# Masthetheus/kmer-ml

Hardware: NVIDIA B200
Metric: kmer_count_feature_throughput (higher is better)
Workload: dtype u32

## Files before the change

### kmerml_b200/csrc/dense.cu

```cuda
#include <algorithm>

#include "fasta_walk.cuh"
#include "internal.h"

namespace km {

struct DevTails {
    const LevelMap* lm;
    GenomeStats* st;
    uint32_t genome;
    __device__ __noinline__ void tail(int j, uint32_t idx) const {
        atomicAdd(lm->ptr(genome, j) + idx, 1u);
        atomicAdd(&st->n_tail[j], 1ull);
    }
};

struct NoTails {
    __device__ __forceinline__ void tail(int, uint32_t) const {}
};

struct TailList {
    unsigned long long* list;
    unsigned int* counts;
    unsigned int* any_full;
// ... 477 lines not shown
    tails.lm = &lm; tails.st = stats + sl.genome; tails.genome = sl.genome;
    Packed16Sink sink;
    sink.sbase = (uint32_t)__cvta_generic_to_shared(sh_hist); sink.n = 0;
    uint32_t* row8 = lm.ptr(sl.genome, 8);
    walk_slice<true, COUNT8_THREADS>(buf, g, sl, P, sink, tails, tc,
                                     [&](uint32_t) { sweep_packed16<COUNT8_THREADS>(sh_hist, row8); });
    const unsigned long long total = block_sum_u32(sink.n, &sh_total);
    for (int i = tid; i < 32768; i += COUNT8_THREADS) packed16_flush_word(sh_hist[i], (uint32_t)i, row8);
    if (tid == 0 && total) atomicAdd(&stats[sl.genome].total_top, total);
}

constexpr int PART_LOW = 7;
constexpr int PART_BINS = 1 << (2 * PART_LOW);
constexpr int PART_MAX_BUCKETS = 1024;
constexpr int PART_SECTOR = 16;

__device__ __noinline__ void overflow_push(uint32_t* ov, unsigned int* ov_count, uint32_t idx) {
    const unsigned act = __activemask();
    const int lane = threadIdx.x & 31;
    const int leader = __ffs(act) - 1;
    unsigned int base = 0;
    if (lane == leader) base = atomicAdd(ov_count, (unsigned int)__popc(act));
    base = __shfl_sync(act, base, leader);
    ov[base + __popc(act & ((1u << lane) - 1u))] = idx;
}

__device__ __forceinline__ uint32_t payload_fix(uint32_t bucket) { return ((bucket & 3u) << 14) * 0x00010001u; }
__device__ __forceinline__ uint32_t payload_pad(uint32_t bucket, uint32_t spread) {
    return (((bucket & 3u) ^ 1u) << 14) | (spread & 255u);
}

__device__ __noinline__ void overflow_push_sector(uint32_t* ov, unsigned int* ov_count, uint32_t bucket,
                                                  const uint16_t* src) {
    for (int i = 0; i < PART_SECTOR; i++)
        overflow_push(ov, ov_count, (bucket << (2 * PART_LOW)) | (src[i] & (uint32_t)(PART_BINS - 1)));
}

template <int NB_SHIFT>
struct PartGeom {
    static constexpr uint32_t nb = 1u << NB_SHIFT;
    static constexpr uint32_t slot_size = NB_SHIFT == 10 ? 48u : (32768u >> NB_SHIFT);
    static constexpr uint32_t stage_entries = nb * slot_size;
    static constexpr bool owned = NB_SHIFT == 10;
};

template <int NB_SHIFT>
struct SlotSink {
    static constexpr bool raw_windows = true;
    static constexpr uint32_t slot_size = PartGeom<NB_SHIFT>::slot_size;
    static constexpr uint32_t b4_mask = (PartGeom<NB_SHIFT>::nb - 1u) << 2;
    uint32_t cnt_s;
    uint32_t staged_s;
    uint32_t* ov;
    unsigned int* ov_count;
    uint32_t kmask;
    unsigned n;
    __device__ __forceinline__ uint32_t atom_inc(uint32_t b4) {
        uint32_t old;
        asm volatile("atom.shared.add.u32 %0, [%1], 1;" : "=r"(old) : "r"(cnt_s + b4) : "memory");
        return old;
    }
    __device__ __forceinline__ void store16(uint32_t b4, uint32_t pos, uint32_t x) {
        const uint32_t e = b4 * (slot_size / 4u) + pos;
        asm volatile("st.shared.u16 [%0], %1;" ::"r"(staged_s + 2u * e), "h"((unsigned short)x) : "memory");
    }
    __device__ __forceinline__ void count(uint32_t idx, uint64_t) {
        const uint32_t b4 = (idx >> (2 * PART_LOW - 2)) & b4_mask;
        const uint32_t pos = atom_inc(b4);
        n++;
        if (pos < slot_size) store16(b4, pos, idx);
        else overflow_push(ov, ov_count, idx);
    }
    __device__ __forceinline__ void count4(uint32_t i0, uint32_t i1, uint32_t i2, uint32_t i3, uint64_t, uint64_t,
                                           uint64_t, uint64_t) {
        count(i0, 0); count(i1, 0); count(i2, 0); count(i3, 0);
    }
    __device__ __forceinline__ void count8(const uint32_t* w, const uint64_t*) { place<8>(w, true); }
    __device__ __forceinline__ void count8_tail(const uint32_t* w, const uint64_t*, bool last) { place<8>(w, last); }
    template <int N>
    __device__ __forceinline__ void place(const uint32_t* x, bool last_live = true) {
        uint32_t b4[N], pos[N];
        bool full = false;
#pragma unroll
        for (int u = 0; u < N; u++) b4[u] = (x[u] >> (2 * PART_LOW - 2)) & b4_mask;
#pragma unroll
        for (int u = 0; u < N; u++) pos[u] = (u < N - 1 || last_live) ? atom_inc(b4[u]) : 0u;
        n += last_live ? N : N - 1;
#pragma unroll
        for (int u = 0; u < N; u++) {
            const bool fits = pos[u] < slot_size;
            full |= !fits;
            if (fits && (u < N - 1 || last_live)) store16(b4[u], pos[u], x[u]);
        }
        if (full) {
#pragma unroll
            for (int u = 0; u < N; u++)
                if (pos[u] >= slot_size) overflow_push(ov, ov_count, x[u] & kmask);
        }
    }
};

struct PartWalkSmem {
    uint32_t last16[COUNT_THREADS];
    uint8_t flags[2 * COUNT_THREADS];
    uint8_t clean[COUNT_THREADS];
};

template <int NB_SHIFT>
struct PartSmem {
    uint16_t staged[PartGeom<NB_SHIFT>::stage_entries];
    uint32_t cnt[PART_MAX_BUCKETS];
    uint16_t written[PART_MAX_BUCKETS];
    PartWalkSmem walk;
    unsigned long long carry[2];
    uint32_t prev_tile[2];
    unsigned long long sh_total;
};
static_assert(sizeof(PartSmem<10>) <= 113 * 1024, "two partition CTAs must fit in one SM's shared memory");

struct GenomeRuns {
    uint32_t run0, n_runs;
};

__device__ __forceinline__ void store_sector(uint4* dst, const uint4& a, const uint4& b) {
    asm volatile("st.global.v8.b32 [%0], {%1, %2, %3, %4, %5, %6, %7, %8};" ::"l"(dst), "r"(a.x), "r"(a.y), "r"(a.z),
                 "r"(a.w), "r"(b.x), "r"(b.y), "r"(b.z), "r"(b.w) : "memory");
}

template <int NB_SHIFT>
__device__ __noinline__ void flush_slot_slow(PartSmem<NB_SHIFT>& sm, uint32_t b, uint4* region, uint32_t cap,
                                             uint32_t* ov, unsigned int* ov_count) {
    constexpr uint32_t slot_size = PartGeom<NB_SHIFT>::slot_size;
    const uint32_t c = min(sm.cnt[b], slot_size);
    const uint32_t nfull = c / PART_SECTOR, left = c % PART_SECTOR;
    uint16_t* slot16 = sm.staged + (size_t)b * slot_size;
    uint4* slot = reinterpret_cast<uint4*>(slot16);
    uint32_t wr = sm.written[b];
    for (uint32_t q = 0; q < nfull; q++) {
        if (wr < cap) {
            region[((size_t)b * cap + wr) * 2] = slot[2 * q];
            region[((size_t)b * cap + wr) * 2 + 1] = slot[2 * q + 1];
            wr++;
        } else {
            overflow_push_sector(ov, ov_count, b, slot16 + q * PART_SECTOR);
        }
    }
    if (nfull && left) {
        const uint4 a = slot[2 * nfull], d = slot[2 * nfull + 1];
        slot[0] = a;
        slot[1] = d;
    }
    sm.written[b] = (uint16_t)wr;
    sm.cnt[b] = left;
}

template <int NB_SHIFT>
__global__ void __launch_bounds__(COUNT_THREADS, 2)
partition_kernel(const uint8_t* __restrict__ buf, const GenomeDev* __restrict__ gds,
                 const Slice* __restrict__ runs, DenseParams P, LevelMap lm,
                 GenomeStats* stats, uint4* __restrict__ payload, uint16_t* __restrict__ nsec, uint32_t cap,
                 uint32_t* __restrict__ overflow, unsigned int* __restrict__ ov_counts, uint64_t batch_lo,
                 TailList tl, int k_stop) {
    using G = PartGeom<NB_SHIFT>;
    constexpr uint32_t slot_size = G::slot_size;
    constexpr uint32_t nb = G::nb;
    constexpr uint32_t VPB = slot_size / 8;
    extern __shared__ __align__(16) unsigned char part_smem_raw[];
    PartSmem<NB_SHIFT>& sm = *reinterpret_cast<PartSmem<NB_SHIFT>*>(part_smem_raw);
    const int tid = threadIdx.x;
    const Slice sl = runs[blockIdx.x];
    const GenomeDev gd = gds[sl.genome];
    Genome g;
    g.b = buf;
    g.lo = gd.lo;
    g.hi = gd.hi;
    TileCtx tc;
    tc.flags = sm.walk.flags; tc.clean = sm.walk.clean; tc.last16 = sm.walk.last16;
    tc.carry = sm.carry; tc.prev_tile = sm.prev_tile;
    for (uint32_t i = tid; i < nb; i += COUNT_THREADS) { sm.cnt[i] = 0; sm.written[i] = 0; }
    if (tid == 0) sm.sh_total = 0;

    SlotSink<NB_SHIFT> sink;
    sink.cnt_s = (uint32_t)__cvta_generic_to_shared(sm.cnt);
    sink.staged_s = (uint32_t)__cvta_generic_to_shared(sm.staged);
    sink.ov = overflow + (gd.file_lo - batch_lo);
    sink.ov_count = ov_counts + sl.genome;
    sink.kmask = P.mask;
    sink.n = 0;
    ListTails tails;
    tails.lm = &lm; tails.st = stats + sl.genome; tails.genome = sl.genome; tails.k_stop = k_stop;
    tails.list = tail_list_of(tl, gd, sl.genome, &tails.cap);
    tails.count = tl.counts + sl.genome;
    tails.any_full = tl.any_full;
    uint4* const region = payload + (size_t)blockIdx.x * nb * cap * 2;
    walk_slice<false>(buf, g, sl, P, sink, tails, tc, [&](uint32_t) {
        uint4* st = reinterpret_cast<uint4*>(sm.staged);
        if (G::owned) {
#pragma unroll
            for (int h = 0; h < 2; h++) {
                const uint32_t b = (uint32_t)tid + h * COUNT_THREADS;
                const uint32_t c = sm.cnt[b];
                if (c < PART_SECTOR) continue;
                const uint32_t wr = sm.written[b];
                if (c > slot_size || wr + 3u > cap) {
                    flush_slot_slow<NB_SHIFT>(sm, b, region, cap, sink.ov, sink.ov_count);
                    continue;
                }
                const uint32_t sw = ((uint32_t)tid >> 2) & 1u, sx = sw ^ 1u;
                uint4* slot = st + b * VPB;
                uint4* dst = region + (b * cap + wr) * 2u;
                {
                    const uint4 x0 = slot[sw], x1 = slot[sx];
                    dst[sw] = x0;
                    dst[sx] = x1;
                }
                uint32_t mv = 2;
                if (c >= 2 * PART_SECTOR) {
                    const uint4 x0 = slot[2 + sw], x1 = slot[2 + sx];
                    dst[2 + sw] = x0;
                    dst[2 + sx] = x1;
                    mv = 4;
                    if (c == 3 * PART_SECTOR) {
                        const uint4 y0 = slot[4 + sw], y1 = slot[4 + sx];
                        dst[4 + sw] = y0;
                        dst[4 + sx] = y1;
                        mv = 0;
                    }
                }
                const uint4 m0 = slot[mv + sw], m1 = slot[mv + sx];
                slot[sw] = m0;
                slot[sx] = m1;
                sm.written[b] = (uint16_t)(wr + c / PART_SECTOR);
                sm.cnt[b] = c % PART_SECTOR;
            }
        } else {
#pragma unroll
            for (int j = 0; j < (int)(G::stage_entries / 8 / COUNT_THREADS); j++) {
                const uint32_t v = (uint32_t)tid + j * COUNT_THREADS;
                const uint32_t b = v / VPB, jv = v % VPB, q = jv >> 1;
                const uint32_t c = min(sm.cnt[b], slot_size);
                const uint32_t nfull = c / PART_SECTOR;
                const uint32_t wr = sm.written[b];
                const uint4 x = st[v];
                if (VPB <= 32) __syncwarp(); else __syncthreads();
                if (q < nfull) {
                    const uint32_t sec = wr + q;
                    if (sec < cap) region[(b * cap + sec) * 2u + (jv & 1u)] = x;
                    else if (!(jv & 1u)) overflow_push_sector(sink.ov, sink.ov_count, b, sm.staged + b * slot_size + q * PART_SECTOR);
                }
                if (VPB <= 32) __syncwarp(); else __syncthreads();
                if (q == nfull && nfull && (c % PART_SECTOR)) st[b * VPB + (jv & 1u)] = x;
                if (jv == 0) {
                    sm.cnt[b] = c % PART_SECTOR;
                    sm.written[b] = (uint16_t)min(wr + nfull, cap);
                }
            }
        }
    });
    __syncthreads();
    for (uint32_t b = tid; b < nb; b += COUNT_THREADS) {
        const uint32_t left = sm.cnt[b];
        uint32_t wr = sm.written[b];
        if (left) {
            uint32_t e[PART_SECTOR / 2];
            const uint16_t* src16 = sm.staged + (size_t)b * slot_size;
            const uint32_t* src = reinterpret_cast<const uint32_t*>(src16);
            if (wr < cap) {
#pragma unroll
                for (int i = 0; i < PART_SECTOR / 2; i++) {
                    uint32_t w = src[i];
                    const uint32_t pad = payload_pad(b, b * 16u + 2u * i);
                    if (2u * i >= left) w = (w & 0xFFFF0000u) | pad;
                    if (2u * i + 1u >= left) w = (w & 0x0000FFFFu) | ((pad ^ 1u) << 16);
                    e[i] = w;
                }
                uint4* dst = region + (b * cap + wr) * 2u;
                dst[0] = make_uint4(e[0], e[1], e[2], e[3]);
                dst[1] = make_uint4(e[4], e[5], e[6], e[7]);
                wr++;
            } else {
                for (uint32_t i = 0; i < left; i++)
                    overflow_push(sink.ov, sink.ov_count, (b << (2 * PART_LOW)) | (src16[i] & (uint32_t)(PART_BINS - 1)));
            }
        }
        nsec[(size_t)blockIdx.x * nb + b] = (uint16_t)wr;
    }
    const unsigned long long total = block_sum_u32(sink.n, &sm.sh_total);
    if (tid == 0 && total) atomicAdd(&stats[sl.genome].total_top, total);
}

struct LevelInfo {
    int ki[16];
};

constexpr int BUCKET_THREADS = 512;

constexpr int BUCKET_NS_CHUNK = 1024;
#ifndef KM_BUCKET_BULK_STORE
#define KM_BUCKET_BULK_STORE 1
#endif
struct BucketSmem {
    uint32_t hist[PART_BINS + 256];
    uint16_t ns[BUCKET_NS_CHUNK];
    unsigned long long tot[16];
    uint32_t* lvl_counts[16];
    float* lvl_freq[16];
    double lvl_inv[16];
};
constexpr int BUCKET_CTAS_PER_SM = 3;
static_assert(sizeof(BucketSmem) <= 75 * 1024, "three bucket CTAs must fit in one SM's shared memory");

__device__ __forceinline__ void bulk_store(void* dst, uint32_t src_smem, uint32_t bytes) {
    asm volatile("cp.async.bulk.global.shared::cta.bulk_group [%0], [%1], %2;" ::"l"(dst), "r"(src_smem), "r"(bytes) : "memory");
    asm volatile("cp.async.bulk.commit_group;" ::: "memory");
}
__device__ __forceinline__ void bulk_store_wait_read() { asm volatile("cp.async.bulk.wait_group.read 0;" ::: "memory"); }

__device__ __forceinline__ void hist_add8(uint32_t hbase, const uint4& x, uint32_t fix) {
    const uint32_t w[4] = {x.x ^ fix, x.y ^ fix, x.z ^ fix, x.w ^ fix};
#pragma unroll
    for (int i = 0; i < 4; i++) {
        asm volatile("red.shared.add.u32 [%0], 1;" ::"r"(hbase + ((w[i] & 0xFFFFu) << 2)) : "memory");
        asm volatile("red.shared.add.u32 [%0], 1;" ::"r"(hbase + ((w[i] >> 16) << 2)) : "memory");
    }
}

__global__ void __launch_bounds__(BUCKET_THREADS, BUCKET_CTAS_PER_SM)
bucket_kernel(LevelMap lm, RowSpec row, LevelInfo li, int k, int k_stop, const GenomeRuns* __restrict__ grs,
              const uint4* __restrict__ payload, const uint16_t* __restrict__ nsec, uint32_t cap,
              const GenomeStats* __restrict__ stats, float* freq, uint64_t freq_stride, uint64_t* totals,
              uint32_t genome0) {
    extern __shared__ __align__(16) unsigned char bucket_smem_raw[];
    BucketSmem& sm = *reinterpret_cast<BucketSmem*>(bucket_smem_raw);
    const int tid = threadIdx.x;
    const uint32_t b = blockIdx.x;
    const uint32_t nb = gridDim.x;
    const uint32_t g = genome0 + blockIdx.y;
    const GenomeRuns gr = grs[g];
    if (tid < row.nk) {
        const int j = row.k[tid];
        unsigned long long t = stats[g].total_top;
        for (int i = j; i < k; i++) t += stats[g].n_tail[i];
        sm.tot[tid] = t;
        if (totals && b == 0) totals[(uint64_t)g * row.nk + tid] = t;
    }
    __syncthreads();
    if (tid >= 32 && tid < 48) {
        const int level = tid - 32;
        uint32_t* cp = nullptr;
        float* fp = nullptr;
        double inv = 0.0;
        if (level >= k_stop && level <= k) {
            const size_t n_level = (size_t)PART_BINS >> (2 * (k - level));
            cp = lm.ptr(g, level) + (size_t)b * n_level;
            const int ki = li.ki[level];
            if (ki >= 0) {
                if (freq) fp = freq + (uint64_t)g * freq_stride + row.off[ki] + (size_t)b * n_level;
                inv = sm.tot[ki] ? 1.0 / (double)sm.tot[ki] : 0.0;
            }
        }
        sm.lvl_counts[level] = cp;
        sm.lvl_freq[level] = fp;
        sm.lvl_inv[level] = inv;
    }
    constexpr int PER1 = PART_BINS / 4 / BUCKET_THREADS;
    constexpr int PER2 = PART_BINS / 16 / BUCKET_THREADS;
    const uint32_t hbase = (uint32_t)__cvta_generic_to_shared(sm.hist);
    const uint32_t fix = payload_fix(b);
    {
        uint4* h4 = reinterpret_cast<uint4*>(sm.hist);
        for (int i = tid; i < (PART_BINS + 256) / 4; i += BUCKET_THREADS) h4[i] = make_uint4(0, 0, 0, 0);
    }
    constexpr int NWARP = BUCKET_THREADS / 32;
    const int lane = tid & 31, wid = tid >> 5;
    const size_t run_stride = (size_t)nb * cap * 2;
    for (uint32_t rb = 0; rb < gr.n_runs; rb += BUCKET_NS_CHUNK) {
        const uint32_t nr = min(gr.n_runs - rb, (uint32_t)BUCKET_NS_CHUNK);
        __syncthreads();
        for (uint32_t i = tid; i < nr; i += BUCKET_THREADS)
            sm.ns[i] = __ldg(nsec + (size_t)(gr.run0 + rb + i) * nb + b);
        __syncthreads();
        const uint4* base = payload + ((size_t)(gr.run0 + rb) * nb + b) * cap * 2;
        uint32_t r = wid, c = 0, nv = 0;
        auto settle = [&]() {
            while (r < nr && 32u * c >= (nv = 2u * sm.ns[r])) { r += NWARP; c = 0; }
        };
        auto issue = [&](uint4& x, bool& live) -> bool {
            settle();
            if (r >= nr) { live = false; return false; }
            const uint32_t v = 32u * c + lane;
            live = v < nv;
            if (live) x = __ldg(base + (size_t)r * run_stride + v);
            c++;
            return true;
        };
        uint4 x0, x1, x2, x3;
        bool l0, l1, l2, l3;
        bool h0 = issue(x0, l0), h1 = issue(x1, l1), h2 = issue(x2, l2), h3 = issue(x3, l3);
        while (h0) {
            if (l0) hist_add8(hbase, x0, fix);
            h0 = issue(x0, l0);
            if (!h1) break;
            if (l1) hist_add8(hbase, x1, fix);
            h1 = issue(x1, l1);
            if (!h2) break;
            if (l2) hist_add8(hbase, x2, fix);
            h2 = issue(x2, l2);
            if (!h3) break;
            if (l3) hist_add8(hbase, x3, fix);
            h3 = issue(x3, l3);
        }
    }
#if KM_BUCKET_BULK_STORE
    asm volatile("fence.proxy.async.shared::cta;" ::: "memory");
    __syncthreads();
    if (tid == 0) bulk_store(sm.lvl_counts[k], hbase, PART_BINS * 4);
#else
    __syncthreads();
#endif
    uint32_t v1r[PER1];
    {
        float* fk = sm.lvl_freq[k];
        const double inv = sm.lvl_inv[k];
        const bool down = k - 1 >= k_stop;
        uint32_t* c1 = down ? sm.lvl_counts[k - 1] : nullptr;
        float* f1 = down ? sm.lvl_freq[k - 1] : nullptr;
        const double inv1 = down ? sm.lvl_inv[k - 1] : 0.0;
#pragma unroll
        for (int u = 0; u < PER1; u++) {
            const int i = tid + u * BUCKET_THREADS;
            const uint4 c = reinterpret_cast<const uint4*>(sm.hist)[i];
#if !KM_BUCKET_BULK_STORE
            reinterpret_cast<uint4*>(sm.lvl_counts[k])[i] = c;
#endif
            if (fk) {
                float4 f;
                f.x = (float)((double)c.x * inv); f.y = (float)((double)c.y * inv);
                f.z = (float)((double)c.z * inv); f.w = (float)((double)c.w * inv);
                reinterpret_cast<float4*>(fk)[i] = f;
            }
            v1r[u] = c.x + c.y + c.z + c.w;
            if (down) {
                c1[i] = v1r[u];
                if (f1) f1[i] = (float)((double)v1r[u] * inv1);
            }
        }
    }
#if KM_BUCKET_BULK_STORE
    if (tid == 0) bulk_store_wait_read();
#endif
    if (k - 2 < k_stop) return;
    __syncthreads();
#pragma unroll
    for (int u = 0; u < PER1; u++) sm.hist[tid + u * BUCKET_THREADS] = v1r[u];
    __syncthreads();
    {
        uint32_t* cl = sm.lvl_counts[k - 2];
        float* fl = sm.lvl_freq[k - 2];
        const double invl = sm.lvl_inv[k - 2];
#pragma unroll
        for (int u = 0; u < PER2; u++) {
            const int i = tid + u * BUCKET_THREADS;
            const uint4 c = reinterpret_cast<const uint4*>(sm.hist)[i];
            const uint32_t v = c.x + c.y + c.z + c.w;
            cl[i] = v;
            if (fl) fl[i] = (float)((double)v * invl);
            sm.hist[4096 + i] = v;
        }
    }
    __syncthreads();
    if (tid >= 32) return;
    uint32_t* cur = sm.hist + 4096;
    uint32_t* nxt = sm.hist + 8192;
    int n_cur = 1024;
    for (int level = k - 3; level >= k_stop; level--) {
        const int n_next = n_cur >> 2;
        uint32_t* cl = sm.lvl_counts[level];
        float* fl = sm.lvl_freq[level];
        const double invl = sm.lvl_inv[level];
        for (int i = tid; i < n_next; i += 32) {
            const uint4 c = reinterpret_cast<const uint4*>(cur)[i];
            const uint32_t v = c.x + c.y + c.z + c.w;
            cl[i] = v;
            if (fl) fl[i] = (float)((double)v * invl);
            nxt[i] = v;
        }
        __syncwarp();
        uint32_t* t = cur; cur = nxt; nxt = t;
        n_cur = n_next;
    }
}

constexpr int OV_TABLE = 4096;
constexpr uint32_t OV_EMPTY = 0xFFFFFFFFu;

__global__ void __launch_bounds__(256)
overflow_kernel(LevelMap lm, RowSpec row, LevelInfo li, int k, int k_stop, const GenomeDev* __restrict__ gds,
                const uint32_t* __restrict__ overflow, const unsigned int* __restrict__ ov_counts, uint64_t batch_lo,
                const GenomeStats* __restrict__ stats, float* freq, uint64_t freq_stride, uint32_t genome0, int pass) {
    __shared__ uint32_t t_key[OV_TABLE];
    __shared__ uint32_t t_cnt[OV_TABLE];
    __shared__ unsigned int t_used;
    const uint32_t g = genome0 + blockIdx.y;
    const unsigned int n = ov_counts[g];
    if (blockIdx.x * 256u >= n) return;
    const uint32_t* ov = overflow + (gds[g].file_lo - batch_lo);
    const int tid = threadIdx.x;
    auto apply = [&](uint32_t idx, uint32_t cnt) {
        for (int level = k; level >= k_stop; level--) {
            const uint32_t x = idx >> (2 * (k - level));
            uint32_t* c = lm.ptr(g, level);
            if (pass == 0) {
                atomicAdd(c + x, cnt);
            } else if (freq && li.ki[level] >= 0) {
                const int ki = li.ki[level];
                unsigned long long t = stats[g].total_top;
                for (int q = level; q < k; q++) t += stats[g].n_tail[q];
                freq[(uint64_t)g * freq_stride + row.off[ki] + x] = t ? (float)((double)c[x] * (1.0 / (double)t)) : 0.0f;
            }
        }
    };
    auto flush = [&]() {
        for (int e = tid; e < OV_TABLE; e += 256) {
            const uint32_t key = t_key[e];
            if (key != OV_EMPTY) apply(key, t_cnt[e]);
            t_key[e] = OV_EMPTY;
            t_cnt[e] = 0;
        }
        if (tid == 0) t_used = 0;
        __syncthreads();
    };
    if (n < 4096u) {
        for (unsigned int i = blockIdx.x * 256u + tid; i < n; i += gridDim.x * 256u) apply(ov[i], 1u);
        return;
    }
    for (int e = tid; e < OV_TABLE; e += 256) { t_key[e] = OV_EMPTY; t_cnt[e] = 0; }
    if (tid == 0) t_used = 0;
    __syncthreads();
    for (unsigned int base = blockIdx.x * 256u; base < n; base += gridDim.x * 256u) {
        const unsigned int i = base + tid;
        if (i < n) {
            const uint32_t idx = ov[i];
            uint32_t h = (idx * 2654435761u) >> 20;
            bool placed = false;
            for (int probe = 0; probe < 8 && !placed; probe++) {
                const uint32_t old = atomicCAS(&t_key[h], OV_EMPTY, idx);
                if (old == OV_EMPTY) atomicAdd(&t_used, 1u);
                if (old == OV_EMPTY || old == idx) {
                    atomicAdd(&t_cnt[h], 1u);
                    placed = true;
                }
                h = (h + 1) & (OV_TABLE - 1);
            }
            if (!placed) apply(idx, 1u);
        }
        __syncthreads();
        const bool crowded = t_used > OV_TABLE / 2;
        __syncthreads();
        if (crowded) flush();
    }
    flush();
}

struct TailApply {
    LevelMap lm;
    RowSpec row;
    LevelInfo li;
    int k, k_stop, pass;
    const GenomeStats* stats;
    float* freq;
    uint64_t freq_stride;
    __device__ __forceinline__ void apply(uint32_t g, int j, uint32_t idx) const {
        for (int level = j; level >= k_stop; level--) {
            const uint32_t x = idx >> (2 * (j - level));
            uint32_t* c = lm.ptr(g, level);
            if (pass == 0) {
                atomicAdd(c + x, 1u);
            } else if (freq && li.ki[level] >= 0) {
                const int ki = li.ki[level];
                unsigned long long t = stats[g].total_top;
                for (int q = level; q < k; q++) t += stats[g].n_tail[q];
                freq[(uint64_t)g * freq_stride + row.off[ki] + x] = t ? (float)((double)c[x] * (1.0 / (double)t)) : 0.0f;
            }
        }
    }
};

__global__ void __launch_bounds__(256)
tails_apply_kernel(TailApply ap, const GenomeDev* __restrict__ gds, TailList tl, uint32_t genome0) {
    const uint32_t g = genome0 + blockIdx.y;
    const unsigned int n = tl.counts[g];
    if (!n) return;
    uint32_t cap;
    const unsigned long long* list = tail_list_of(tl, gds[g], g, &cap);
    if (n > cap) return;
    for (unsigned int i = blockIdx.x * 256 + threadIdx.x; i < n; i += gridDim.x * 256) {
        const unsigned long long e = list[i];
        ap.apply(g, (int)(e >> 32), (uint32_t)e);
    }
}

struct NullSink {
    __device__ __forceinline__ void count(uint32_t, uint64_t) {}
    __device__ __forceinline__ void count4(uint32_t, uint32_t, uint32_t, uint32_t, uint64_t, uint64_t, uint64_t, uint64_t) {}
    __device__ __forceinline__ void count8(const uint32_t*, const uint64_t*) {}
    __device__ __forceinline__ void count8_tail(const uint32_t*, const uint64_t*, bool) {}
};
struct RescanTails {
    const TailApply* ap;
    uint32_t genome;
    __device__ __noinline__ void tail(int j, uint32_t idx) const {
        if (j >= ap->k_stop) ap->apply(genome, j, idx);
    }
};

__global__ void __launch_bounds__(COUNT_THREADS)
tails_rescan_kernel(const uint8_t* __restrict__ buf, const GenomeDev* __restrict__ gds, const Slice* __restrict__ slices,
                    int n_slices, DenseParams P, TailApply ap, TailList tl) {
    if (*tl.any_full == 0) return;
    KM_TILE_SMEM(rs)
    for (int i = blockIdx.x; i < n_slices; i += gridDim.x) {
        const Slice sl = slices[i];
        const GenomeDev gd = gds[sl.genome];
        uint32_t cap;
        (void)tail_list_of(tl, gd, sl.genome, &cap);
        if (tl.counts[sl.genome] <= cap) continue;
        Genome g;
        g.b = buf;
        g.lo = gd.lo;
        g.hi = gd.hi;
        NullSink sink;
        RescanTails tails;
        tails.ap = &ap; tails.genome = sl.genome;
        walk_slice<true>(buf, g, sl, P, sink, tails, tc, [](uint32_t) {});
        __syncthreads();
    }
}

__global__ void __launch_bounds__(256)
finalize_low_kernel(LevelMap lm, RowSpec row, int k_top, int level_limit, const GenomeStats* __restrict__ stats,
                    float* freq, uint64_t freq_stride, uint32_t genome0) {
    __shared__ unsigned long long tot[16];
    const uint32_t g = genome0 + blockIdx.x;
    level_totals(row, k_top, stats, g, tot, nullptr, false);
    if (!freq) return;
    for (int ki = 0; ki < row.nk; ki++) {
        const int j = row.k[ki];
        if (j >= level_limit) continue;
        const uint32_t* c = lm.ptr(g, j);
        float* f = freq + (uint64_t)g * freq_stride + row.off[ki];
        const double inv = tot[ki] ? 1.0 / (double)tot[ki] : 0.0;
        for (uint32_t x = threadIdx.x; x < (1u << (2 * j)); x += 256) f[x] = (float)((double)c[x] * inv);
    }
}

__global__ void __launch_bounds__(256)
cascade_kernel(LevelMap lm, int k_top, int depth, uint32_t genome0) {
    __shared__ uint32_t sh[256];
    const int tid = threadIdx.x;
    const uint32_t g = genome0 + blockIdx.y;
    const uint64_t n2 = k_top >= 2 ? 1ull << (2 * (k_top - 2)) : 0;
    const uint64_t q2 = (uint64_t)blockIdx.x * 256 + tid;
    uint32_t w = 0;
    if (k_top >= 2 ? q2 < n2 : q2 == 0) {
        const uint4* hi = reinterpret_cast<const uint4*>(lm.ptr(g, k_top)) + 4 * q2;
        uint4 h0 = hi[0], h1 = hi[1], h2 = hi[2], h3 = hi[3];
        uint4* lo1 = reinterpret_cast<uint4*>(lm.ptr(g, k_top - 1)) + q2;
        uint4 t = *lo1;
        t.x += h0.x + h0.y + h0.z + h0.w;
        t.y += h1.x + h1.y + h1.z + h1.w;
        t.z += h2.x + h2.y + h2.z + h2.w;
        t.w += h3.x + h3.y + h3.z + h3.w;
        *lo1 = t;
        if (depth >= 2) {
            uint32_t* lo2 = lm.ptr(g, k_top - 2);
            w = t.x + t.y + t.z + t.w + lo2[q2];
            lo2[q2] = w;
        }
    }
    if (depth < 3) return;
    sh[tid] = w;
    __syncthreads();
    int width = 256;
    for (int d = 3; d <= depth; d++) {
        width >>= 2;
        const int level = k_top - d;
        uint32_t nv = 0;
        if (tid < width) {
            const uint64_t q = (uint64_t)blockIdx.x * width + tid;
            if (q < (1ull << (2 * level))) {
                uint32_t* lo = lm.ptr(g, level);
                nv = sh[4 * tid] + sh[4 * tid + 1] + sh[4 * tid + 2] + sh[4 * tid + 3] + lo[q];
                lo[q] = nv;
            }
        }
        __syncthreads();
// ... 379 lines not shown
```

Measured before the change: 251.2.

## Balance bucket histogram work across warps via prefix-summed round counts

Replaces the round-robin assignment of runs to warps with a block-wide prefix sum over per-run 32-lane rounds. Each warp then takes an equal contiguous slice of the total rounds and binary-searches for its starting run. This targets load imbalance when run lengths vary, where some warps finish early while others process long runs. The cost is an extra scan with a sync, a small binary search, and more shared memory per CTA, which could pressure the three-CTAs-per-SM budget.

```diff
diff --git a/kmerml_b200/csrc/dense.cu b/kmerml_b200/csrc/dense.cu
--- a/kmerml_b200/csrc/dense.cu
+++ b/kmerml_b200/csrc/dense.cu
@@ -803,6 +803,8 @@
 struct BucketSmem {
     uint32_t hist[PART_BINS + 256];
     uint16_t ns[BUCKET_NS_CHUNK];
+    uint32_t rounds[BUCKET_NS_CHUNK + 1];
+    uint32_t warp_rounds[BUCKET_THREADS / 32];
     unsigned long long tot[16];
     uint32_t* lvl_counts[16];
     float* lvl_freq[16];
@@ -866,6 +868,7 @@
     }
     constexpr int PER1 = PART_BINS / 4 / BUCKET_THREADS;
     constexpr int PER2 = PART_BINS / 16 / BUCKET_THREADS;
+    static_assert(BUCKET_NS_CHUNK == 2 * BUCKET_THREADS, "a thread counts the rounds of two runs");
     const uint32_t hbase = (uint32_t)__cvta_generic_to_shared(sm.hist);
     const uint32_t fix = payload_fix(b);
     {
@@ -878,21 +881,55 @@
     for (uint32_t rb = 0; rb < gr.n_runs; rb += BUCKET_NS_CHUNK) {
         const uint32_t nr = min(gr.n_runs - rb, (uint32_t)BUCKET_NS_CHUNK);
         __syncthreads();
-        for (uint32_t i = tid; i < nr; i += BUCKET_THREADS)
-            sm.ns[i] = __ldg(nsec + (size_t)(gr.run0 + rb + i) * nb + b);
+        uint32_t ra = 0, rbr = 0;
+        if (2u * tid < nr) {
+            const uint32_t n = __ldg(nsec + (size_t)(gr.run0 + rb + 2u * tid) * nb + b);
+            sm.ns[2 * tid] = (uint16_t)n;
+            ra = (2u * n + 31u) / 32u;
+        }
+        if (2u * tid + 1u < nr) {
+            const uint32_t n = __ldg(nsec + (size_t)(gr.run0 + rb + 2u * tid + 1u) * nb + b);
+            sm.ns[2 * tid + 1] = (uint16_t)n;
+            rbr = (2u * n + 31u) / 32u;
+        }
+        uint32_t x = ra + rbr;
+#pragma unroll
+        for (int o = 1; o < 32; o <<= 1) {
+            const uint32_t y = __shfl_up_sync(0xffffffffu, x, o);
+            if (lane >= o) x += y;
+        }
+        if (lane == 31) sm.warp_rounds[wid] = x;
+        __syncthreads();
+        uint32_t before = x - ra - rbr, n_rounds = 0;
+#pragma unroll
+        for (int w = 0; w < NWARP; w++) {
+            const uint32_t t = sm.warp_rounds[w];
+            before += w < wid ? t : 0u;
+            n_rounds += t;
+        }
+        if (2u * tid < nr) sm.rounds[2 * tid + 1] = before + ra;
+        if (2u * tid + 1u < nr) sm.rounds[2 * tid + 2] = before + ra + rbr;
+        if (tid == 0) sm.rounds[0] = 0;
         __syncthreads();
         const uint4* base = payload + ((size_t)(gr.run0 + rb) * nb + b) * cap * 2;
-        uint32_t r = wid, c = 0, nv = 0;
-        auto settle = [&]() {
-            while (r < nr && 32u * c >= (nv = 2u * sm.ns[r])) { r += NWARP; c = 0; }
-        };
+        uint32_t i = (uint32_t)(((uint64_t)n_rounds * wid) / NWARP);
+        const uint32_t end = (uint32_t)(((uint64_t)n_rounds * (wid + 1)) / NWARP);
+        uint32_t r = 0;
+        for (uint32_t step = BUCKET_NS_CHUNK / 2; step; step >>= 1)
+            if (r + step < nr && sm.rounds[r + step] <= i) r += step;
+        uint32_t r_lo = sm.rounds[r], r_hi = sm.rounds[r + 1], nv = 2u * sm.ns[r];
         auto issue = [&](uint4& x, bool& live) -> bool {
-            settle();
-            if (r >= nr) { live = false; return false; }
-            const uint32_t v = 32u * c + lane;
+            if (i >= end) { live = false; return false; }
+            while (i >= r_hi) {
+                r++;
+                r_lo = r_hi;
+                r_hi = sm.rounds[r + 1];
+                nv = 2u * sm.ns[r];
+            }
+            const uint32_t v = 32u * (i - r_lo) + lane;
             live = v < nv;
             if (live) x = __ldg(base + (size_t)r * run_stride + v);
-            c++;
+            i++;
             return true;
         };
         uint4 x0, x1, x2, x3;
```

After: 252.0, median of 6. No clear change (+0.3%).
